# psmyth94/mamba-clip

Hardware: AMD Instinct MI355X
Metric: image-text pairs/sec (whole node) + selective_scan HBM GB/s (higher is better)
Workload: dtype bf16; 1 GPU; C2: ViT-B/16 image + Mamba-130M text, contrastive train step (fwd+bwd+AdamW), amp_bf16; model=vit_b16-mamba130m, global_batch=256, per_gpu_batch=256, seq_len=77, image_size=224, input=resident, step_launch=eager, parallelism=dp1, library_gemm_selection=tunableop-file

## Files before the change

### include/mc_ops.h

```cpp
#ifndef MAMBA_CLIP_AMD_MC_OPS_H
#define MAMBA_CLIP_AMD_MC_OPS_H

#include <stddef.h>
#include <stdint.h>

#include "mc_scan.h"

#ifdef __cplusplus
extern "C" {
#endif

int mc_add_rmsnorm_fwd(int32_t rows, int32_t cols, int32_t dtype, const void* x, const float* res_in, const float* w,
                       float eps, void* y, float* res_out, float* rstd, void* stream);

int mc_add_rmsnorm_bwd(int32_t rows, int32_t cols, int32_t dtype, const void* dy, const float* dres, const float* h,
                       const float* w, const float* rstd, void* dx, float* dres_in, float* dw, void* workspace,
                       size_t workspace_bytes, void* stream);
size_t mc_add_rmsnorm_bwd_workspace_bytes(int32_t rows, int32_t cols);

int mc_last_token_rmsnorm_fwd(int32_t batch, int32_t T, int32_t Lp, int32_t cols, int32_t dtype, const int64_t* tokens,
                              int64_t pad_id, const void* x, const float* res_in, const float* w, float eps, void* y,
                              float* h_out, float* rstd, int32_t* pos, void* stream);

int mc_last_token_rmsnorm_bwd(int32_t batch, int32_t Lp, int32_t cols, int32_t dtype, const void* dy, const float* h,
// ... 29 lines not shown
  const float* scale;
  const float* shift;
  void* out;
} mc_patch_input_params;
int mc_patch_embed_input(const mc_patch_input_params* p, void* stream);

size_t mc_grad_colsum_workspace_bytes(int32_t rows, int32_t cols);
int mc_gelu_bwd(int32_t rows, int32_t cols, int32_t dtype, const void* h, int64_t ldh, const void* ga, int64_t ldga,
                void* gh, int64_t ldgh, float* dbias, void* workspace, size_t workspace_bytes, void* stream);

typedef struct mc_qkv_pack_params {
  int32_t batch, seq, heads, head_dim, dtype;
  const void* src[3];
  int64_t sb[3], sn[3], sh[3];
  void* out; int64_t ld_out;
  float* dbias;
  void* workspace; size_t workspace_bytes;
} mc_qkv_pack_params;
int mc_qkv_grad_pack(const mc_qkv_pack_params* p, void* stream);

int mc_stream_copy(const void* src, void* dst, size_t nbytes, void* stream);

int mc_sum_slabs(int32_t s, int64_t n, const float* src, int64_t slab_stride, float* dst, void* stream);

#define MC_CAST_CHUNK 16384
typedef struct {
  const float* src;
  int64_t dst_off;
  int64_t n;
} mc_cast_chunk;
int mc_cast_f32_many(int32_t n_chunks, const mc_cast_chunk* chunks, void* dst_base, int32_t dst_dtype, void* stream);

typedef struct mc_cast_t_tile {
  const float* src;
  int64_t dst_off;
  int32_t src_ld, dst_ld;
  int32_t rows, cols;
} mc_cast_t_tile;
int mc_cast_transpose_f32_many(int32_t n_tiles, const mc_cast_t_tile* tiles, void* dst_base, int32_t dst_dtype,
                               void* stream);

#define MC_ADAMW_MAX_GROUPS 8
#define MC_ADAMW_CHUNK 65536
typedef struct mc_adamw_tensor {
  float* p;
  float* m;
  float* v;
  const float* g;
} mc_adamw_tensor;
typedef struct mc_adamw_chunk {
  int32_t tensor, group;
  int64_t off, n;
} mc_adamw_chunk;
typedef struct mc_adamw_group {
  float beta1, beta2, eps, decay;
  float step_size, bc2_sqrt;
} mc_adamw_group;
typedef struct mc_adamw_hyper {
  int32_t n_groups, reserved;
  mc_adamw_group group[MC_ADAMW_MAX_GROUPS];
} mc_adamw_hyper;
int mc_adamw_step(int32_t n_chunks, const mc_adamw_chunk* chunks, const mc_adamw_tensor* tensors,
                  const mc_adamw_hyper* hyper, void* stream);

size_t mc_colsum_workspace_bytes(int32_t rows, int32_t cols);
int mc_colsum(int32_t rows, int32_t cols, int32_t dtype, const void* x, int64_t ld, float* out,
              void* workspace, size_t workspace_bytes, void* stream);
int mc_colsum_fold(int32_t nslices, int32_t cols, const float* part, float* out, void* stream);

int mc_l2norm_fwd(int32_t rows, int32_t cols, int32_t dtype, const void* x, int64_t ldx, float eps,
                  float* y, int64_t ldy, float* norm, void* stream);
int mc_l2norm_bwd(int32_t rows, int32_t cols, int32_t dtype, const void* x, int64_t ldx, const float* norm,
                  float eps, const float* g, int64_t ldg, void* dx, int64_t lddx, void* stream);

#ifdef __cplusplus
}
#endif
#endif
```

### mamba-clip_amd/csrc/ops.hip

```cpp
#include <algorithm>

#include "mc_common.h"
#include "../../include/mc_ops.h"

namespace mc {

namespace ops {

constexpr int kMaxVec = 8;

template <int V>
__device__ __forceinline__ void ld_f32v(const float* __restrict__ p, float (&v)[V]) {
#pragma unroll
  for (int e4 = 0; e4 < V; e4 += 4) {
    const float4 q = *reinterpret_cast<const float4*>(p + e4);
    v[e4] = q.x; v[e4 + 1] = q.y; v[e4 + 2] = q.z; v[e4 + 3] = q.w;
  }
}
template <int V>
__device__ __forceinline__ void st_f32v(float* __restrict__ p, const float (&v)[V]) {
#pragma unroll
  for (int e4 = 0; e4 < V; e4 += 4)
    *reinterpret_cast<float4*>(p + e4) = make_float4(v[e4], v[e4 + 1], v[e4 + 2], v[e4 + 3]);
}

template <int V>
__device__ __forceinline__ void fold_stage(float (&red)[3][64 * V], const float (&acc)[V], int lane) {
  const int w = threadIdx.x >> 6;
  if (w > 0) {
#pragma unroll
    for (int e = 0; e < V; ++e) red[w - 1][lane * V + e] = acc[e];
  }
  __syncthreads();
// ... 1356 lines not shown
  if (vec) {
    for (int64_t i = 8 * (int64_t)threadIdx.x; i < c.n; i += 8 * 256) {
      const float4 a = *reinterpret_cast<const float4*>(c.src + i);
      const float4 b = *reinterpret_cast<const float4*>(c.src + i + 4);
      const float v[8] = {a.x, a.y, a.z, a.w, b.x, b.y, b.z, b.w};
      *reinterpret_cast<uint4*>(dst + i) = pack_f<TO>(v);
    }
  } else {
    for (int64_t i = threadIdx.x; i < c.n; i += 256) dst[i] = from_f<TO>(c.src[i]);
  }
}
}

extern "C" int mc_cast_f32_many(int32_t n_chunks, const mc_cast_chunk* chunks, void* dst_base, int32_t dst_dtype,
                                void* stream) {
  MC_CHECK(n_chunks >= 0 && (n_chunks == 0 || (chunks && dst_base)), MC_ERR_INVALID, "mc_cast_f32_many: bad chunk table");
  MC_CHECK(dst_dtype == MC_DTYPE_BF16 || dst_dtype == MC_DTYPE_F16, MC_ERR_DTYPE,
           "mc_cast_f32_many: dst dtype %d (bf16 / f16 only)", dst_dtype);
  if (n_chunks == 0) return MC_OK;
  if (dst_dtype == MC_DTYPE_BF16)
    hipLaunchKernelGGL(cast_many_kernel<bf16_t>, dim3(n_chunks), dim3(256), 0, (hipStream_t)stream, chunks,
                       reinterpret_cast<bf16_t*>(dst_base));
  else
    hipLaunchKernelGGL(cast_many_kernel<f16_t>, dim3(n_chunks), dim3(256), 0, (hipStream_t)stream, chunks,
                       reinterpret_cast<f16_t*>(dst_base));
  return check_launch("mc_cast_f32_many");
}

namespace {
template <typename TO>
__global__ __launch_bounds__(256) void cast_transpose_kernel(const mc_cast_t_tile* __restrict__ tiles, TO* __restrict__ base) {
  __shared__ float tile[64][65];
  const mc_cast_t_tile t = tiles[blockIdx.x];
  const int tid = threadIdx.x, r = tid >> 2, a = tid & 3;
  const bool full = t.rows == 64 && t.cols == 64 && (t.src_ld & 3) == 0 && (reinterpret_cast<uintptr_t>(t.src) & 15) == 0;
  if (full) {
    float4 v[4];
#pragma unroll
    for (int k = 0; k < 4; ++k) v[k] = *reinterpret_cast<const float4*>(t.src + (int64_t)r * t.src_ld + 4 * (a + 4 * k));
#pragma unroll
    for (int k = 0; k < 4; ++k) {
      const int c = 4 * (a + 4 * k);
      tile[r][c] = v[k].x; tile[r][c + 1] = v[k].y; tile[r][c + 2] = v[k].z; tile[r][c + 3] = v[k].w;
    }
  } else {
#pragma unroll
    for (int k = 0; k < 4; ++k)
#pragma unroll
      for (int e = 0; e < 4; ++e) {
        const int c = 4 * (a + 4 * k) + e;
        tile[r][c] = (r < t.rows && c < t.cols) ? t.src[(int64_t)r * t.src_ld + c] : 0.f;
      }
  }
  __syncthreads();
  const int j = tid >> 2;
  TO* dst = base + t.dst_off + (int64_t)j * t.dst_ld;
  const bool vec = full && (t.dst_ld & 7) == 0 && (reinterpret_cast<uintptr_t>(base + t.dst_off) & 15) == 0;
#pragma unroll
  for (int hlf = 0; hlf < 2; ++hlf) {
    const int g = a + 4 * hlf;
    float v[8];
#pragma unroll
    for (int e = 0; e < 8; ++e) v[e] = tile[8 * g + e][j];
    if (vec) {
      *reinterpret_cast<uint4*>(dst + 8 * g) = pack_f<TO>(v);
    } else if (j < t.cols) {
#pragma unroll
      for (int e = 0; e < 8; ++e)
        if (8 * g + e < t.rows) dst[8 * g + e] = from_f<TO>(v[e]);
    }
  }
}
}

extern "C" int mc_cast_transpose_f32_many(int32_t n_tiles, const mc_cast_t_tile* tiles, void* dst_base, int32_t dst_dtype,
                                          void* stream) {
  MC_CHECK(n_tiles >= 0 && (n_tiles == 0 || (tiles && dst_base)), MC_ERR_INVALID, "mc_cast_transpose_f32_many: bad tile table");
  MC_CHECK(dst_dtype == MC_DTYPE_BF16 || dst_dtype == MC_DTYPE_F16, MC_ERR_DTYPE,
           "mc_cast_transpose_f32_many: dst dtype %d (bf16 / f16 only)", dst_dtype);
  if (n_tiles == 0) return MC_OK;
  if (dst_dtype == MC_DTYPE_BF16)
    hipLaunchKernelGGL(cast_transpose_kernel<bf16_t>, dim3(n_tiles), dim3(256), 0, (hipStream_t)stream, tiles,
                       reinterpret_cast<bf16_t*>(dst_base));
  else
    hipLaunchKernelGGL(cast_transpose_kernel<f16_t>, dim3(n_tiles), dim3(256), 0, (hipStream_t)stream, tiles,
                       reinterpret_cast<f16_t*>(dst_base));
  return check_launch("mc_cast_transpose_f32_many");
}

namespace {
__device__ __forceinline__ void adamw_elem(float& p, float& m, float& v, float g, const mc_adamw_group& h) {
  p *= h.decay;
  m = h.beta1 * m + (1.f - h.beta1) * g;
  v = h.beta2 * v + (1.f - h.beta2) * g * g;
  const float denom = sqrtf(v) / h.bc2_sqrt + h.eps;
  p -= h.step_size * m / denom;
}

__global__ __launch_bounds__(256) void adamw_kernel(const mc_adamw_chunk* __restrict__ chunks,
                                                    const mc_adamw_tensor* __restrict__ tensors, const mc_adamw_hyper hy) {
  const mc_adamw_chunk c = chunks[blockIdx.x];
  const mc_adamw_tensor t = tensors[c.tensor];
  const mc_adamw_group h = hy.group[c.group];
  float* __restrict__ p = t.p + c.off;
  float* __restrict__ m = t.m + c.off;
  float* __restrict__ v = t.v + c.off;
  const float* __restrict__ g = t.g + c.off;
  const bool vec = ((reinterpret_cast<uintptr_t>(p) | reinterpret_cast<uintptr_t>(m) | reinterpret_cast<uintptr_t>(v) |
                     reinterpret_cast<uintptr_t>(g)) & 15) == 0;
  const int64_t n4 = vec ? c.n / 4 : 0;
  for (int64_t i = threadIdx.x; i < n4; i += 256) {
    float4 pp = reinterpret_cast<float4*>(p)[i], mm = reinterpret_cast<float4*>(m)[i];
    float4 vv = reinterpret_cast<float4*>(v)[i];
    const float4 gg = reinterpret_cast<const float4*>(g)[i];
    adamw_elem(pp.x, mm.x, vv.x, gg.x, h);
    adamw_elem(pp.y, mm.y, vv.y, gg.y, h);
    adamw_elem(pp.z, mm.z, vv.z, gg.z, h);
    adamw_elem(pp.w, mm.w, vv.w, gg.w, h);
    reinterpret_cast<float4*>(p)[i] = pp;
    reinterpret_cast<float4*>(m)[i] = mm;
    reinterpret_cast<float4*>(v)[i] = vv;
  }
  for (int64_t i = 4 * n4 + threadIdx.x; i < c.n; i += 256) {
    float pp = p[i], mm = m[i], vv = v[i];
    adamw_elem(pp, mm, vv, g[i], h);
    p[i] = pp;
    m[i] = mm;
    v[i] = vv;
  }
}
}

extern "C" int mc_adamw_step(int32_t n_chunks, const mc_adamw_chunk* chunks, const mc_adamw_tensor* tensors,
                             const mc_adamw_hyper* hyper, void* stream) {
  MC_CHECK(n_chunks >= 0 && hyper, MC_ERR_INVALID, "mc_adamw_step: bad arguments");
  MC_CHECK(hyper->n_groups >= 1 && hyper->n_groups <= MC_ADAMW_MAX_GROUPS, MC_ERR_INVALID,
           "mc_adamw_step: n_groups %d (1..%d)", hyper->n_groups, MC_ADAMW_MAX_GROUPS);
  if (n_chunks == 0) return MC_OK;
  MC_CHECK(chunks && tensors, MC_ERR_INVALID, "mc_adamw_step: null chunk / tensor table");
  hipLaunchKernelGGL(adamw_kernel, dim3(n_chunks), dim3(256), 0, (hipStream_t)stream, chunks, tensors, *hyper);
  return check_launch("mc_adamw_step");
}

namespace {
template <bool kVec>
__global__ __launch_bounds__(256) void sum_slabs_kernel(int s, int64_t n, const float* __restrict__ src, int64_t stride,
                                                        float* __restrict__ dst) {
  const int64_t i0 = ((int64_t)blockIdx.x * 256 + threadIdx.x) * (kVec ? 4 : 1);
  if (i0 >= n) return;
  if constexpr (kVec) {
    float4 acc = *reinterpret_cast<const float4*>(src + i0);
    for (int k = 1; k < s; ++k) {
      const float4 v = *reinterpret_cast<const float4*>(src + (int64_t)k * stride + i0);
      acc.x += v.x; acc.y += v.y; acc.z += v.z; acc.w += v.w;
    }
    *reinterpret_cast<float4*>(dst + i0) = acc;
  } else {
    float acc = src[i0];
    for (int k = 1; k < s; ++k) acc += src[(int64_t)k * stride + i0];
    dst[i0] = acc;
  }
}
}

extern "C" int mc_sum_slabs(int32_t s, int64_t n, const float* src, int64_t slab_stride, float* dst, void* stream) {
  MC_CHECK(s >= 1 && n >= 0 && slab_stride >= n, MC_ERR_SHAPE, "mc_sum_slabs: bad shape (s %d, n %lld, stride %lld)", s,
           (long long)n, (long long)slab_stride);
  if (n == 0) return MC_OK;
  MC_CHECK(src && dst, MC_ERR_INVALID, "mc_sum_slabs: null pointer");
  const bool vec = n % 4 == 0 && slab_stride % 4 == 0 && aligned16(src) && aligned16(dst);
  const int64_t items = vec ? n / 4 : n;
  const dim3 grid((unsigned)((items + 255) / 256));
  if (vec) hipLaunchKernelGGL(sum_slabs_kernel<true>, grid, dim3(256), 0, (hipStream_t)stream, s, n, src, slab_stride, dst);
  else hipLaunchKernelGGL(sum_slabs_kernel<false>, grid, dim3(256), 0, (hipStream_t)stream, s, n, src, slab_stride, dst);
// ... 69 lines not shown
```

### mamba-clip_amd/mamba_clip_amd/_lib.py

```python
import ctypes
import os

_HERE = os.path.dirname(os.path.abspath(__file__))
LIB_PATH = os.environ.get("MAMBA_CLIP_AMD_LIB") or os.path.join(_HERE, "libmamba_clip_amd.so")

MC_DTYPE_F32, MC_DTYPE_BF16, MC_DTYPE_F16, MC_DTYPE_FP8_E4M3, MC_DTYPE_U8 = 0, 1, 2, 3, 4
MC_LAYOUT_NCHW, MC_LAYOUT_NHWC = 0, 1
MC_SCAN_CHUNK = 32
MC_SCAN_STATE_INTERVAL_FINE = 8
MC_SCAN_KERNEL_NONE, MC_SCAN_KERNEL_PAIR, MC_SCAN_KERNEL_GENERIC, MC_SCAN_KERNEL_DIRS = 0, 1, 2, 3
MC_GEMM_KERNEL_TILE, MC_GEMM_KERNEL_FP8_TILE, MC_GEMM_KERNEL_FP8_PANEL = 1, 2, 3
MC_SCAN_MAX_DSTATE = 32
MC_CAST_CHUNK = 16384

c_i32, c_i64, c_vp, c_fp = ctypes.c_int32, ctypes.c_int64, ctypes.c_void_p, ctypes.c_void_p


class ScanFwdParams(ctypes.Structure):
    _fields_ = [
        ("batch", c_i32), ("dim", c_i32), ("seqlen", c_i32), ("dstate", c_i32), ("n_groups", c_i32),
        ("itype", c_i32), ("wtype", c_i32), ("delta_softplus", c_i32),
        ("u_batch_stride", c_i64), ("u_dim_stride", c_i64),
        ("delta_batch_stride", c_i64), ("delta_dim_stride", c_i64),
        ("z_batch_stride", c_i64), ("z_dim_stride", c_i64),
# ... 238 lines not shown
    "mc_retrieval_ranks_workspace_bytes": (ctypes.c_size_t, [c_i32, c_i32]),
    "mc_sigmoid_loss_fwd": (ctypes.c_int, [ctypes.POINTER(SigmoidLossParams), c_vp]),
    "mc_sigmoid_loss_fwd_workspace_bytes": (ctypes.c_size_t, [c_i32, c_i32]),
    "mc_sigmoid_loss_grad": (ctypes.c_int, [ctypes.POINTER(SigmoidLossParams), c_vp]),
    "mc_sigmoid_loss_grad_workspace_bytes": (ctypes.c_size_t, [c_i32, c_i32]),
    "mc_add_rmsnorm_fwd": (ctypes.c_int, [c_i32, c_i32, c_i32, c_vp, c_fp, c_fp, ctypes.c_float, c_vp, c_fp, c_fp,
                                          c_vp]),
    "mc_add_rmsnorm_bwd": (ctypes.c_int, [c_i32, c_i32, c_i32, c_vp, c_fp, c_fp, c_fp, c_fp, c_vp, c_fp, c_fp, c_vp,
                                          ctypes.c_size_t, c_vp]),
    "mc_add_rmsnorm_bwd_workspace_bytes": (ctypes.c_size_t, [c_i32, c_i32]),
    "mc_last_token_rmsnorm_fwd": (ctypes.c_int, [c_i32, c_i32, c_i32, c_i32, c_i32, c_vp, c_i64, c_vp, c_fp, c_fp,
                                                 ctypes.c_float, c_vp, c_fp, c_fp, c_vp, c_vp]),
    "mc_last_token_rmsnorm_bwd": (ctypes.c_int, [c_i32, c_i32, c_i32, c_i32, c_vp, c_fp, c_fp, c_fp, c_vp, c_vp, c_fp,
                                                 c_fp, c_vp]),
    "mc_add_layernorm_fwd": (ctypes.c_int, [c_i32, c_i32, c_i32, c_vp, c_vp, c_fp, c_fp, ctypes.c_float, c_vp, c_vp,
                                            c_fp, c_fp, c_vp]),
    "mc_add_layernorm_bwd": (ctypes.c_int, [c_i32, c_i32, c_i32, c_vp, c_vp, c_vp, c_fp, c_fp, c_fp, c_vp, c_fp, c_fp,
                                            c_fp, c_vp, ctypes.c_size_t, c_vp]),
    "mc_add_layernorm_bwd_workspace_bytes": (ctypes.c_size_t, [c_i32, c_i32]),
    "mc_causal_conv1d_fwd": (ctypes.c_int, [c_i32, c_i32, c_i32, c_i32, c_i32, c_vp, c_i64, c_i64, c_fp, c_fp, c_i32,
                                            c_vp, c_i64, c_i64, c_vp]),
    "mc_causal_conv1d_bwd": (ctypes.c_int, [c_i32, c_i32, c_i32, c_i32, c_i32, c_vp, c_i64, c_i64, c_fp, c_fp, c_i32,
                                            c_vp, c_i64, c_i64, c_vp, c_i64, c_i64, c_fp, c_fp, c_vp,
                                            ctypes.c_size_t, c_vp]),
    "mc_causal_conv1d_bwd_workspace_bytes": (ctypes.c_size_t, [c_i32, c_i32, c_i32, c_i32]),
    "mc_patch_im2col": (ctypes.c_int, [c_i32, c_i32, c_i32, c_i32, c_i32, c_i32, c_vp, c_vp, c_vp]),
    "mc_grad_colsum_workspace_bytes": (ctypes.c_size_t, [c_i32, c_i32]),
    "mc_gelu_bwd": (ctypes.c_int, [c_i32, c_i32, c_i32, c_vp, c_i64, c_vp, c_i64, c_vp, c_i64, c_fp, c_vp,
                                   ctypes.c_size_t, c_vp]),
    "mc_qkv_grad_pack": (ctypes.c_int, [ctypes.POINTER(QkvPackParams), c_vp]),
    "mc_stream_copy": (ctypes.c_int, [c_vp, c_vp, ctypes.c_size_t, c_vp]),
    "mc_cast_f32_many": (ctypes.c_int, [c_i32, c_vp, c_vp, c_i32, c_vp]),
    "mc_cast_transpose_f32_many": (ctypes.c_int, [c_i32, c_vp, c_vp, c_i32, c_vp]),
    "mc_adamw_step": (ctypes.c_int, [c_i32, c_vp, c_vp, ctypes.POINTER(AdamWHyper), c_vp]),
    "mc_sum_slabs": (ctypes.c_int, [c_i32, c_i64, c_fp, c_i64, c_fp, c_vp]),
    "mc_colsum_workspace_bytes": (ctypes.c_size_t, [c_i32, c_i32]),
    "mc_colsum_fold": (ctypes.c_int, [c_i32, c_i32, c_fp, c_fp, c_vp]),
    "mc_colsum": (ctypes.c_int, [c_i32, c_i32, c_i32, c_vp, c_i64, c_fp, c_vp, ctypes.c_size_t, c_vp]),
    "mc_l2norm_fwd": (ctypes.c_int, [c_i32, c_i32, c_i32, c_vp, c_i64, ctypes.c_float, c_fp, c_i64, c_fp, c_vp]),
    "mc_l2norm_bwd": (ctypes.c_int, [c_i32, c_i32, c_i32, c_vp, c_i64, c_fp, ctypes.c_float, c_fp, c_i64, c_vp,
                                     c_i64, c_vp]),
    "mc_attn_fwd": (ctypes.c_int, [ctypes.POINTER(AttnFwdParams), c_vp]),
    "mc_attn_bwd": (ctypes.c_int, [ctypes.POINTER(AttnBwdParams), c_vp]),
    "mc_attn_masked_fwd": (ctypes.c_int, [ctypes.POINTER(AttnMaskedFwdParams), c_vp]),
    "mc_attn_masked_bwd": (ctypes.c_int, [ctypes.POINTER(AttnMaskedBwdParams), c_vp]),
    "mc_patch_embed_input": (ctypes.c_int, [ctypes.POINTER(PatchInputParams), c_vp]),
    "mc_ss2d_conv_stack_fwd": (ctypes.c_int, [ctypes.POINTER(SS2DConvParams), c_vp]),
    "mc_ss2d_conv_stack_bwd": (ctypes.c_int, [ctypes.POINTER(SS2DConvBwdParams), c_vp]),
    "mc_ss2d_conv_bwd_workspace_bytes": (ctypes.c_size_t, [c_i32, c_i32, c_i32, c_i32, c_i32]),
    "mc_ss2d_merge_ln_gate_fwd": (ctypes.c_int, [ctypes.POINTER(SS2DMergeParams), c_vp]),
    "mc_ss2d_merge_ln_gate_bwd": (ctypes.c_int, [ctypes.POINTER(SS2DMergeBwdParams), c_vp]),
    "mc_ss2d_merge_bwd_workspace_bytes": (ctypes.c_size_t, [c_i32, c_i32, c_i32, c_i32]),
    "mc_ss2d_group_proj": (ctypes.c_int, [ctypes.POINTER(SS2DGroupProjParams), c_vp]),
}

_lib = None


def load():
    global _lib
    if _lib is not None:
        return _lib
    if not os.path.exists(LIB_PATH):
        raise ImportError(
            f"mamba_clip_amd: HIP library not found at {LIB_PATH}; build it with "
            "`make -C mamba-clip_amd` (gfx950).  There is no CPU fallback.")
    import torch
# ... 32 lines not shown
```

### mamba-clip_amd/mamba_clip_amd/ops.py

```python
import collections
import ctypes
import weakref

import torch

from . import _lib


def _ws(nbytes, device):
    return torch.empty(max(int(nbytes), 16), dtype=torch.uint8, device=device)


def gemm_nt(A, B, alpha=1.0, alpha_dev=None, out_dtype=torch.float32, scale_a=None, scale_b=None, out=None):
    lib = _lib.load()
    if A.dtype != B.dtype or A.dtype not in (torch.bfloat16, torch.float32, torch.float8_e4m3fn):
        raise RuntimeError("gemm_nt: A and B must both be bf16, both fp32 or both float8_e4m3fn")
    if A.stride(-1) != 1:
        A = A.contiguous()
    if B.stride(-1) != 1:
        B = B.contiguous()
    M, K = A.shape
    N, K2 = B.shape
    if K != K2:
        raise RuntimeError("gemm_nt: inner dimensions differ")
# ... 918 lines not shown
        ctx.save_for_backward(*outs)
        ctx.set_materialize_grads(False)
        return tuple(outs)

    @staticmethod
    def backward(ctx, *gs):
        outs = ctx.saved_tensors
        idx = [i for i, g in enumerate(gs) if g is not None]
        res = [None] * len(gs)
        if idx:
            for i, v in zip(idx, torch._foreach_mul([gs[i].float() for i in idx], [outs[i] for i in idx])):
                res[i] = v
        return tuple(res)


def neg_exp_many(logs):
    return list(NegExpManyFn.apply(*logs))


class GradHandoff:

    def __init__(self):
        self.du = None

    def take(self):
        du, self.du = self.du, None
        return du


_WCAST = None
_WCAST_T = None
_T_WANTED = weakref.WeakValueDictionary()
_CAST_PLANS = {}


def _wcast(t, dt):
    if t.dtype == dt:
        return t
    if _WCAST is not None:
        e = _WCAST.get(id(t))
        if e is not None and e[0] is t and e[1].dtype == dt:
            return e[1]
    return t.to(dt)


class _CastPlan:

    def __init__(self, params, dt, device):
        offs, off = [], 0
        rows = []
        for p in params:
            offs.append(off)
            n = p.numel()
            for s0 in range(0, n, _lib.MC_CAST_CHUNK):
                rows.append((p.data_ptr() + 4 * s0, off + s0, min(_lib.MC_CAST_CHUNK, n - s0)))
            off += (n + 7) // 8 * 8
        self.offs, self.total, self.dt = offs, off, dt
        self.nchunks = len(rows)
        self.table = torch.tensor(rows, dtype=torch.int64).to(device)

    def run(self, params):
        buf = torch.empty(self.total, device=self.table.device, dtype=self.dt)
        _lib.check(_lib.load().mc_cast_f32_many(self.nchunks, self.table.data_ptr(), buf.data_ptr(),
                                                _lib.dtype_code(self.dt), _lib.stream_handle(buf.device)),
                   "mc_cast_f32_many")
        return [buf[o:o + p.numel()].view(p.shape) for o, p in zip(self.offs, params)]


def _wcast_t(weight, x, dt):
    if not (x.is_cuda and weight.dim() == 2 and weight.numel() >= 1 << 19
            and x.numel() // max(x.shape[-1], 1) >= 8192):
        return None
    if _WCAST_T is not None:
        e = _WCAST_T.get(id(weight))
        if e is not None and e[0] is weight and e[1].dtype == dt:
            return e[1]
    if _WCAST is not None and weight.dtype == torch.float32:
        _T_WANTED[id(weight)] = weight
    return None


class _TransposePlan:

    def __init__(self, params, dt, device):
        offs, off, rows = [], 0, []
        for p in params:
            R, C = p.shape
            offs.append(off)
            for r0 in range(0, R, 64):
                for c0 in range(0, C, 64):
                    rows.append((p.data_ptr() + 4 * (r0 * C + c0), off + c0 * R + r0,
                                 C | (R << 32), min(64, R - r0) | (min(64, C - c0) << 32)))
            off += (R * C + 7) // 8 * 8
        self.offs, self.total, self.dt = offs, off, dt
        self.ntiles = len(rows)
        self.table = torch.tensor(rows, dtype=torch.int64).to(device)

    def run(self, params):
        buf = torch.empty(self.total, device=self.table.device, dtype=self.dt)
        _lib.check(_lib.load().mc_cast_transpose_f32_many(self.ntiles, self.table.data_ptr(), buf.data_ptr(),
                                                          _lib.dtype_code(self.dt), _lib.stream_handle(buf.device)),
                   "mc_cast_transpose_f32_many")
        return [buf[o:o + p.numel()].view(p.shape[1], p.shape[0]) for o, p in zip(self.offs, params)]


class weight_cast_scope:

    def __init__(self, module, dt):
        self.module, self.dt, self.active = module, dt, False

    def __enter__(self):
        global _WCAST, _WCAST_T
        if _WCAST is not None or self.dt not in (torch.bfloat16, torch.float16):
            return self
        params = [p for m in self.module.modules() if isinstance(m, torch.nn.Linear)
                  for p in (m.weight, m.bias)
                  if p is not None and p.is_cuda and p.dtype == torch.float32 and p.is_contiguous()]
        if not params:
            return self
        key = (id(self.module), self.dt, tuple((p.data_ptr(), p.numel()) for p in params))
        plan = _CAST_PLANS.get(key[:2])
        if plan is None or plan[0] != key:
            plan = (key, _CastPlan(params, self.dt, params[0].device))
            _CAST_PLANS[key[:2]] = plan
        copies = plan[1].run(params)
        _WCAST = {id(p): (p, c) for p, c in zip(params, copies)}
        tparams = [p for p in params if p.dim() == 2 and _T_WANTED.get(id(p)) is p]
        if tparams:
            tkey = (id(self.module), self.dt, "t", tuple((p.data_ptr(), p.shape) for p in tparams))
            tplan = _CAST_PLANS.get(tkey[:3])
            if tplan is None or tplan[0] != tkey:
                tplan = (tkey, _TransposePlan(tparams, self.dt, params[0].device))
                _CAST_PLANS[tkey[:3]] = tplan
            tcopies = tplan[1].run(tparams)
            _WCAST_T = {id(p): (p, c) for p, c in zip(tparams, tcopies)}
        self.active = True
        return self

    def __exit__(self, *exc):
        global _WCAST, _WCAST_T
        if self.active:
            _WCAST = _WCAST_T = None
        return False


def _dgrad(g2, wc, wt=None):
    if wt is not None:
        return torch.mm(g2, wt.t())
    if g2.is_cuda and g2.shape[0] >= 8192 and wc.shape[0] * wc.shape[1] >= 1 << 19:
        return torch.mm(g2, wc.t().contiguous().t())
    return torch.mm(g2, wc)


def _compute_dtype(t):
    if t.is_cuda and torch.is_autocast_enabled("cuda"):
        return torch.get_autocast_dtype("cuda")
    return t.dtype


class LinearSK(torch.autograd.Function):

    @staticmethod
    def forward(ctx, x, weight, bias):
        dt = _compute_dtype(x)
        xc, wc = x.to(dt), _wcast(weight, dt)
# ... 616 lines not shown
```

### mamba-clip_amd/mamba_clip_amd/optim.py

```python
import math

import torch

from . import _lib


class HipAdamW(torch.optim.Optimizer):
    def __init__(self, params, lr=1e-3, betas=(0.9, 0.999), eps=1e-8, weight_decay=1e-2):
        if not 0.0 <= lr or not 0.0 <= eps or not 0.0 <= betas[0] < 1.0 or not 0.0 <= betas[1] < 1.0:
            raise ValueError(f"HipAdamW: invalid hyper-parameters lr={lr} betas={betas} eps={eps}")
        super().__init__(params, dict(lr=lr, betas=betas, eps=eps, weight_decay=weight_decay, amsgrad=False,
                                      maximize=False, foreach=None, capturable=False, differentiable=False,
                                      fused=None, decoupled_weight_decay=True))
        self._plans = {}

    def _share_steps(self):
        for group in self.param_groups:
            shared = {}
            for p in group["params"]:
                s = self.state.get(p)
                if s is None or "step" not in s:
                    continue
                t = float(s["step"])
                if t not in shared:
                    shared[t] = torch.tensor(t, dtype=torch.float32)
                s["step"] = shared[t]

    def load_state_dict(self, state_dict):
        super().load_state_dict(state_dict)
        self._share_steps()
        self._plans = {}

    def state_dict(self):
        sd = super().state_dict()
        sd["state"] = {k: dict(v, step=v["step"].clone()) if "step" in v else v for k, v in sd["state"].items()}
        return sd

    def _advance_steps(self, group, ps):
        movers = {}
        fresh = []
        for p in ps:
            s = self.state[p]
            if "exp_avg" not in s:
                s["exp_avg"] = torch.zeros_like(p, memory_format=torch.preserve_format)
                s["exp_avg_sq"] = torch.zeros_like(p, memory_format=torch.preserve_format)
            st = s.get("step")
            if st is None:
                fresh.append(s)
            else:
                movers.setdefault(id(st), (st, []))[1].append(s)
        if fresh:
            one = torch.tensor(1.0, dtype=torch.float32)
            for s in fresh:
                s["step"] = one
        if not movers:
            return
        holders = {}
        for p in group["params"]:
            st = self.state.get(p, {}).get("step")
            if st is not None and id(st) in movers:
                holders[id(st)] = holders.get(id(st), 0) + 1
        for key, (st, states) in movers.items():
            if len(states) == holders[key]:
                st += 1.0
            else:
                nxt = st + 1.0
                for s in states:
                    s["step"] = nxt

    @staticmethod
    def _build_plan(live, dev):
        chunks, tensors = [], []
        for ti, (bi, p, s) in enumerate(live):
            n = p.numel()
            for off in range(0, n, _lib.MC_ADAMW_CHUNK):
                chunks.append((ti | (bi << 32), off, min(_lib.MC_ADAMW_CHUNK, n - off)))
            tensors.append((p.data_ptr(), s["exp_avg"].data_ptr(), s["exp_avg_sq"].data_ptr()))
        return dict(n=len(chunks), chunks=torch.tensor(chunks, dtype=torch.int64).to(dev), base=tensors)

    @torch.no_grad()
    def step(self, closure=None):
        loss = None
        if closure is not None:
            with torch.enable_grad():
                loss = closure()
        buckets = {}
        for gi, group in enumerate(self.param_groups):
            if group.get("amsgrad") or group.get("maximize") or not group.get("decoupled_weight_decay", True):
                raise RuntimeError("HipAdamW: amsgrad / maximize / coupled weight decay are not supported")
            ps = [p for p in group["params"] if p.grad is not None]
            for p in ps:
                if p.grad.is_sparse:
                    raise RuntimeError("HipAdamW does not support sparse gradients")
                if not (p.is_cuda and p.dtype == torch.float32 and p.is_contiguous()
                        and p.grad.dtype == torch.float32 and p.grad.is_contiguous()):
                    raise RuntimeError("HipAdamW: fp32 contiguous CUDA parameters and gradients only")
            self._advance_steps(group, ps)
            for p in ps:
                s = self.state[p]
                buckets.setdefault((gi, float(s["step"])), []).append((p, s))
        if not buckets:
            return loss
        keys = list(buckets)
        per = _lib.MC_ADAMW_MAX_GROUPS
        for b0 in range(0, len(keys), per):
            self._launch([(k, buckets[k]) for k in keys[b0:b0 + per]])
        return loss

    def _launch(self, bucket_list):
        hyper = _lib.AdamWHyper()
        hyper.n_groups = len(bucket_list)
        live = []
        for bi, ((gi, t), members) in enumerate(bucket_list):
            group = self.param_groups[gi]
            b1, b2 = group["betas"]
            h = hyper.group[bi]
            h.beta1, h.beta2, h.eps = b1, b2, group["eps"]
            h.decay = 1.0 - group["lr"] * group["weight_decay"]
            h.step_size = group["lr"] / (1.0 - b1 ** t)
            h.bc2_sqrt = math.sqrt(1.0 - b2 ** t)
            live.extend((bi, p, s) for p, s in members)
        dev = live[0][1].device
        key = tuple((bi, id(p), p.data_ptr(), id(s["exp_avg"])) for bi, p, s in live)
        plan = self._plans.get(key)
        if plan is None:
            if len(self._plans) > 16:
                self._plans.clear()
            plan = self._plans[key] = self._build_plan(live, dev)
        rows = [b + (p.grad.data_ptr(),) for b, (_, p, _) in zip(plan["base"], live)]
        tens = torch.tensor(rows, dtype=torch.int64).pin_memory().to(dev, non_blocking=True)
        _lib.check(_lib.load().mc_adamw_step(plan["n"], plan["chunks"].data_ptr(), tens.data_ptr(), hyper,
                                             _lib.stream_handle(dev)), "mc_adamw_step")
        plan["tens"] = tens
```

Measured before the change: 3766 image-text pairs/sec.

## Emit bf16 weight shadows from AdamW and reuse them for forward casts

The AdamW kernel now also writes a low-precision copy of each updated parameter into a persistent shadow buffer. The forward-pass weight cast then reuses these shadows instead of re-reading fp32 weights and casting them again. Transposed weight copies are built by a new 16-bit transpose kernel that reads the shadows instead of cast-transposing from fp32. This removes a separate fp32 read and cast pass per step, at the cost of extra shadow memory and version-tracking bookkeeping that must stay correct when parameters change outside the optimizer.

```diff
diff --git a/include/mc_ops.h b/include/mc_ops.h
--- a/include/mc_ops.h
+++ b/include/mc_ops.h
@@ -85,13 +85,14 @@
 int mc_cast_f32_many(int32_t n_chunks, const mc_cast_chunk* chunks, void* dst_base, int32_t dst_dtype, void* stream);
 
 typedef struct mc_cast_t_tile {
-  const float* src;
+  const void* src;
   int64_t dst_off;
   int32_t src_ld, dst_ld;
   int32_t rows, cols;
 } mc_cast_t_tile;
 int mc_cast_transpose_f32_many(int32_t n_tiles, const mc_cast_t_tile* tiles, void* dst_base, int32_t dst_dtype,
                                void* stream);
+int mc_transpose16_many(int32_t n_tiles, const mc_cast_t_tile* tiles, void* dst_base, int32_t dtype, void* stream);
 
 #define MC_ADAMW_MAX_GROUPS 8
 #define MC_ADAMW_CHUNK 65536
@@ -115,6 +116,8 @@
 } mc_adamw_hyper;
 int mc_adamw_step(int32_t n_chunks, const mc_adamw_chunk* chunks, const mc_adamw_tensor* tensors,
                   const mc_adamw_hyper* hyper, void* stream);
+int mc_adamw_step_shadow(int32_t n_chunks, const mc_adamw_chunk* chunks, const mc_adamw_tensor* tensors,
+                         void* const* shadows, int32_t shadow_dtype, const mc_adamw_hyper* hyper, void* stream);
 
 size_t mc_colsum_workspace_bytes(int32_t rows, int32_t cols);
 int mc_colsum(int32_t rows, int32_t cols, int32_t dtype, const void* x, int64_t ld, float* out,
diff --git a/mamba-clip_amd/csrc/ops.hip b/mamba-clip_amd/csrc/ops.hip
--- a/mamba-clip_amd/csrc/ops.hip
+++ b/mamba-clip_amd/csrc/ops.hip
@@ -1,4 +1,5 @@
 #include <algorithm>
+#include <type_traits>
 
 #include "mc_common.h"
 #include "../../include/mc_ops.h"
@@ -1421,12 +1422,13 @@
 __global__ __launch_bounds__(256) void cast_transpose_kernel(const mc_cast_t_tile* __restrict__ tiles, TO* __restrict__ base) {
   __shared__ float tile[64][65];
   const mc_cast_t_tile t = tiles[blockIdx.x];
+  const float* __restrict__ src = static_cast<const float*>(t.src);
   const int tid = threadIdx.x, r = tid >> 2, a = tid & 3;
-  const bool full = t.rows == 64 && t.cols == 64 && (t.src_ld & 3) == 0 && (reinterpret_cast<uintptr_t>(t.src) & 15) == 0;
+  const bool full = t.rows == 64 && t.cols == 64 && (t.src_ld & 3) == 0 && (reinterpret_cast<uintptr_t>(src) & 15) == 0;
   if (full) {
     float4 v[4];
 #pragma unroll
-    for (int k = 0; k < 4; ++k) v[k] = *reinterpret_cast<const float4*>(t.src + (int64_t)r * t.src_ld + 4 * (a + 4 * k));
+    for (int k = 0; k < 4; ++k) v[k] = *reinterpret_cast<const float4*>(src + (int64_t)r * t.src_ld + 4 * (a + 4 * k));
 #pragma unroll
     for (int k = 0; k < 4; ++k) {
       const int c = 4 * (a + 4 * k);
@@ -1438,7 +1440,7 @@
 #pragma unroll
       for (int e = 0; e < 4; ++e) {
         const int c = 4 * (a + 4 * k) + e;
-        tile[r][c] = (r < t.rows && c < t.cols) ? t.src[(int64_t)r * t.src_ld + c] : 0.f;
+        tile[r][c] = (r < t.rows && c < t.cols) ? src[(int64_t)r * t.src_ld + c] : 0.f;
       }
   }
   __syncthreads();
@@ -1460,6 +1462,67 @@
     }
   }
 }
+
+__global__ __launch_bounds__(256) void transpose16_kernel(const mc_cast_t_tile* __restrict__ tiles,
+                                                          uint16_t* __restrict__ base) {
+  __shared__ uint16_t tile[64][66];
+  const mc_cast_t_tile t = tiles[blockIdx.x];
+  const uint16_t* __restrict__ src = static_cast<const uint16_t*>(t.src);
+  const int tid = threadIdx.x, r = tid >> 2, a = tid & 3;
+  const bool full = t.rows == 64 && t.cols == 64 && (t.src_ld & 7) == 0 && (reinterpret_cast<uintptr_t>(src) & 15) == 0;
+  if (full) {
+    uint4 v[2];
+#pragma unroll
+    for (int k = 0; k < 2; ++k) v[k] = *reinterpret_cast<const uint4*>(src + (int64_t)r * t.src_ld + 8 * (a + 4 * k));
+#pragma unroll
+    for (int k = 0; k < 2; ++k) {
+      const int c = 8 * (a + 4 * k);
+#pragma unroll
+      for (int w = 0; w < 4; ++w) {
+        const uint32_t x = word_of(v[k], w);
+        tile[r][c + 2 * w] = (uint16_t)(x & 0xffffu);
+        tile[r][c + 2 * w + 1] = (uint16_t)(x >> 16);
+      }
+    }
+  } else {
+#pragma unroll
+    for (int k = 0; k < 2; ++k)
+#pragma unroll
+      for (int e = 0; e < 8; ++e) {
+        const int c = 8 * (a + 4 * k) + e;
+        tile[r][c] = (r < t.rows && c < t.cols) ? src[(int64_t)r * t.src_ld + c] : (uint16_t)0;
+      }
+  }
+  __syncthreads();
+  const int j = tid >> 2;
+  uint16_t* dst = base + t.dst_off + (int64_t)j * t.dst_ld;
+  const bool vec = full && (t.dst_ld & 7) == 0 && (reinterpret_cast<uintptr_t>(base + t.dst_off) & 15) == 0;
+#pragma unroll
+  for (int hlf = 0; hlf < 2; ++hlf) {
+    const int g = a + 4 * hlf;
+    uint32_t v[8];
+#pragma unroll
+    for (int e = 0; e < 8; ++e) v[e] = tile[8 * g + e][j];
+    if (vec) {
+      *reinterpret_cast<uint4*>(dst + 8 * g) =
+          make_uint4(v[0] | (v[1] << 16), v[2] | (v[3] << 16), v[4] | (v[5] << 16), v[6] | (v[7] << 16));
+    } else if (j < t.cols) {
+#pragma unroll
+      for (int e = 0; e < 8; ++e)
+        if (8 * g + e < t.rows) dst[8 * g + e] = (uint16_t)v[e];
+    }
+  }
+}
+}
+
+extern "C" int mc_transpose16_many(int32_t n_tiles, const mc_cast_t_tile* tiles, void* dst_base, int32_t dtype, void* stream) {
+  MC_CHECK(n_tiles >= 0 && (n_tiles == 0 || (tiles && dst_base)), MC_ERR_INVALID, "mc_transpose16_many: bad tile table");
+  MC_CHECK(dtype == MC_DTYPE_BF16 || dtype == MC_DTYPE_F16, MC_ERR_DTYPE, "mc_transpose16_many: dtype %d (bf16 / f16 only)",
+           dtype);
+  if (n_tiles == 0) return MC_OK;
+  hipLaunchKernelGGL(transpose16_kernel,dim3(n_tiles), dim3(256), 0, (hipStream_t)stream, tiles,
+                     reinterpret_cast<uint16_t*>(dst_base));
+  return check_launch("mc_transpose16_many");
 }
 
 extern "C" int mc_cast_transpose_f32_many(int32_t n_tiles, const mc_cast_t_tile* tiles, void* dst_base, int32_t dst_dtype,
@@ -1486,11 +1549,9 @@
   p -= h.step_size * m / denom;
 }
 
-__global__ __launch_bounds__(256) void adamw_kernel(const mc_adamw_chunk* __restrict__ chunks,
-                                                    const mc_adamw_tensor* __restrict__ tensors, const mc_adamw_hyper hy) {
-  const mc_adamw_chunk c = chunks[blockIdx.x];
-  const mc_adamw_tensor t = tensors[c.tensor];
-  const mc_adamw_group h = hy.group[c.group];
+template <typename TS>
+__device__ __forceinline__ void adamw_chunk(const mc_adamw_chunk& c, const mc_adamw_tensor& t, void* shadow,
+                                            const mc_adamw_group& h) {
   float* __restrict__ p = t.p + c.off;
   float* __restrict__ m = t.m + c.off;
   float* __restrict__ v = t.v + c.off;
@@ -1498,37 +1559,115 @@
   const bool vec = ((reinterpret_cast<uintptr_t>(p) | reinterpret_cast<uintptr_t>(m) | reinterpret_cast<uintptr_t>(v) |
                      reinterpret_cast<uintptr_t>(g)) & 15) == 0;
   const int64_t n4 = vec ? c.n / 4 : 0;
-  for (int64_t i = threadIdx.x; i < n4; i += 256) {
-    float4 pp = reinterpret_cast<float4*>(p)[i], mm = reinterpret_cast<float4*>(m)[i];
-    float4 vv = reinterpret_cast<float4*>(v)[i];
-    const float4 gg = reinterpret_cast<const float4*>(g)[i];
-    adamw_elem(pp.x, mm.x, vv.x, gg.x, h);
-    adamw_elem(pp.y, mm.y, vv.y, gg.y, h);
-    adamw_elem(pp.z, mm.z, vv.z, gg.z, h);
-    adamw_elem(pp.w, mm.w, vv.w, gg.w, h);
-    reinterpret_cast<float4*>(p)[i] = pp;
-    reinterpret_cast<float4*>(m)[i] = mm;
-    reinterpret_cast<float4*>(v)[i] = vv;
-  }
-  for (int64_t i = 4 * n4 + threadIdx.x; i < c.n; i += 256) {
-    float pp = p[i], mm = m[i], vv = v[i];
-    adamw_elem(pp, mm, vv, g[i], h);
-    p[i] = pp;
-    m[i] = mm;
-    v[i] = vv;
-  }
+  if constexpr (std::is_void<TS>::value) {
+    for (int64_t i = threadIdx.x; i < n4; i += 256) {
+      float4 pp = reinterpret_cast<float4*>(p)[i], mm = reinterpret_cast<float4*>(m)[i];
+      float4 vv = reinterpret_cast<float4*>(v)[i];
+      const float4 gg = reinterpret_cast<const float4*>(g)[i];
+      adamw_elem(pp.x, mm.x, vv.x, gg.x, h);
+      adamw_elem(pp.y, mm.y, vv.y, gg.y, h);
+      adamw_elem(pp.z, mm.z, vv.z, gg.z, h);
+      adamw_elem(pp.w, mm.w, vv.w, gg.w, h);
+      reinterpret_cast<float4*>(p)[i] = pp;
+      reinterpret_cast<float4*>(m)[i] = mm;
+      reinterpret_cast<float4*>(v)[i] = vv;
+    }
+    for (int64_t i = 4 * n4 + threadIdx.x; i < c.n; i += 256) {
+      float pp = p[i], mm = m[i], vv = v[i];
+      adamw_elem(pp, mm, vv, g[i], h);
+      p[i] = pp;
+      m[i] = mm;
+      v[i] = vv;
+    }
+  } else {
+    TS* __restrict__ sh = shadow ? static_cast<TS*>(shadow) + c.off : nullptr;
+    const bool sh8 = (reinterpret_cast<uintptr_t>(sh) & 7) == 0;
+    for (int64_t i = threadIdx.x; i < n4; i += 256) {
+      float4 pp = reinterpret_cast<float4*>(p)[i], mm = reinterpret_cast<float4*>(m)[i];
+      float4 vv = reinterpret_cast<float4*>(v)[i];
+      const float4 gg = reinterpret_cast<const float4*>(g)[i];
+      adamw_elem(pp.x, mm.x, vv.x, gg.x, h);
+      adamw_elem(pp.y, mm.y, vv.y, gg.y, h);
+      adamw_elem(pp.z, mm.z, vv.z, gg.z, h);
+      adamw_elem(pp.w, mm.w, vv.w, gg.w, h);
+      reinterpret_cast<float4*>(p)[i] = pp;
+      reinterpret_cast<float4*>(m)[i] = mm;
+      reinterpret_cast<float4*>(v)[i] = vv;
+      if (sh) {
+        if (sh8) {
+          reinterpret_cast<uint2*>(sh)[i] = make_uint2(cvt_pk2<TS>(pp.x, pp.y), cvt_pk2<TS>(pp.z, pp.w));
+        } else {
+          sh[4 * i] = from_f<TS>(pp.x);
+          sh[4 * i + 1] = from_f<TS>(pp.y);
+          sh[4 * i + 2] = from_f<TS>(pp.z);
+          sh[4 * i + 3] = from_f<TS>(pp.w);
+        }
+      }
+    }
+    for (int64_t i = 4 * n4 + threadIdx.x; i < c.n; i += 256) {
+      float pp = p[i], mm = m[i], vv = v[i];
+      adamw_elem(pp, mm, vv, g[i], h);
+      p[i] = pp;
+      m[i] = mm;
+      v[i] = vv;
+    }
+    if (sh)
+      for (int64_t i = 4 * n4 + threadIdx.x; i < c.n; i += 256) sh[i] = from_f<TS>(p[i]);
+  }
+}
+
+__global__ __launch_bounds__(256) void adamw_kernel(const mc_adamw_chunk* __restrict__ chunks,
+                                                    const mc_adamw_tensor* __restrict__ tensors, const mc_adamw_hyper hy) {
+  const mc_adamw_chunk c = chunks[blockIdx.x];
+  const mc_adamw_tensor t = tensors[c.tensor];
+  const mc_adamw_group h = hy.group[c.group];
+  adamw_chunk<void>(c, t, nullptr, h);
+}
+
+template <typename TS>
+__global__ __launch_bounds__(256) void adamw_shadow_kernel(const mc_adamw_chunk* __restrict__ chunks,
+                                                           const mc_adamw_tensor* __restrict__ tensors,
+                                                           void* const* __restrict__ shadows, const mc_adamw_hyper hy) {
+  const mc_adamw_chunk c = chunks[blockIdx.x];
+  const mc_adamw_tensor t = tensors[c.tensor];
+  const mc_adamw_group h = hy.group[c.group];
+  adamw_chunk<TS>(c, t, shadows[c.tensor], h);
+}
+}
+
+namespace {
+int adamw_check(int32_t n_chunks, const mc_adamw_hyper* hyper, const char* who) {
+  MC_CHECK(n_chunks >= 0 && hyper, MC_ERR_INVALID, "%s: bad arguments", who);
+  MC_CHECK(hyper->n_groups >= 1 && hyper->n_groups <= MC_ADAMW_MAX_GROUPS, MC_ERR_INVALID, "%s: n_groups %d (1..%d)", who,
+           hyper->n_groups, MC_ADAMW_MAX_GROUPS);
+  return MC_OK;
 }
 }
 
 extern "C" int mc_adamw_step(int32_t n_chunks, const mc_adamw_chunk* chunks, const mc_adamw_tensor* tensors,
                              const mc_adamw_hyper* hyper, void* stream) {
-  MC_CHECK(n_chunks >= 0 && hyper, MC_ERR_INVALID, "mc_adamw_step: bad arguments");
-  MC_CHECK(hyper->n_groups >= 1 && hyper->n_groups <= MC_ADAMW_MAX_GROUPS, MC_ERR_INVALID,
-           "mc_adamw_step: n_groups %d (1..%d)", hyper->n_groups, MC_ADAMW_MAX_GROUPS);
+  if (const int rc = adamw_check(n_chunks, hyper, "mc_adamw_step")) return rc;
   if (n_chunks == 0) return MC_OK;
   MC_CHECK(chunks && tensors, MC_ERR_INVALID, "mc_adamw_step: null chunk / tensor table");
   hipLaunchKernelGGL(adamw_kernel, dim3(n_chunks), dim3(256), 0, (hipStream_t)stream, chunks, tensors, *hyper);
   return check_launch("mc_adamw_step");
+}
+
+extern "C" int mc_adamw_step_shadow(int32_t n_chunks, const mc_adamw_chunk* chunks, const mc_adamw_tensor* tensors,
+                                    void* const* shadows, int32_t shadow_dtype, const mc_adamw_hyper* hyper, void* stream) {
+  if (!shadows) return mc_adamw_step(n_chunks, chunks, tensors, hyper, stream);
+  if (const int rc = adamw_check(n_chunks, hyper, "mc_adamw_step_shadow")) return rc;
+  MC_CHECK(shadow_dtype == MC_DTYPE_BF16 || shadow_dtype == MC_DTYPE_F16, MC_ERR_DTYPE,
+           "mc_adamw_step_shadow: shadow dtype %d (bf16 / f16 only)", shadow_dtype);
+  if (n_chunks == 0) return MC_OK;
+  MC_CHECK(chunks && tensors, MC_ERR_INVALID, "mc_adamw_step_shadow: null chunk / tensor table");
+  if (shadow_dtype == MC_DTYPE_BF16)
+    hipLaunchKernelGGL(adamw_shadow_kernel<bf16_t>, dim3(n_chunks), dim3(256), 0, (hipStream_t)stream, chunks, tensors,
+                       shadows, *hyper);
+  else
+    hipLaunchKernelGGL(adamw_shadow_kernel<f16_t>, dim3(n_chunks), dim3(256), 0, (hipStream_t)stream, chunks, tensors,
+                       shadows, *hyper);
+  return check_launch("mc_adamw_step_shadow");
 }
 
 namespace {
diff --git a/mamba-clip_amd/mamba_clip_amd/_lib.py b/mamba-clip_amd/mamba_clip_amd/_lib.py
--- a/mamba-clip_amd/mamba_clip_amd/_lib.py
+++ b/mamba-clip_amd/mamba_clip_amd/_lib.py
@@ -294,7 +294,9 @@
     "mc_stream_copy": (ctypes.c_int, [c_vp, c_vp, ctypes.c_size_t, c_vp]),
     "mc_cast_f32_many": (ctypes.c_int, [c_i32, c_vp, c_vp, c_i32, c_vp]),
     "mc_cast_transpose_f32_many": (ctypes.c_int, [c_i32, c_vp, c_vp, c_i32, c_vp]),
+    "mc_transpose16_many": (ctypes.c_int, [c_i32, c_vp, c_vp, c_i32, c_vp]),
     "mc_adamw_step": (ctypes.c_int, [c_i32, c_vp, c_vp, ctypes.POINTER(AdamWHyper), c_vp]),
+    "mc_adamw_step_shadow": (ctypes.c_int, [c_i32, c_vp, c_vp, c_vp, c_i32, ctypes.POINTER(AdamWHyper), c_vp]),
     "mc_sum_slabs": (ctypes.c_int, [c_i32, c_i64, c_fp, c_i64, c_fp, c_vp]),
     "mc_colsum_workspace_bytes": (ctypes.c_size_t, [c_i32, c_i32]),
     "mc_colsum_fold": (ctypes.c_int, [c_i32, c_i32, c_fp, c_fp, c_vp]),
diff --git a/mamba-clip_amd/mamba_clip_amd/ops.py b/mamba-clip_amd/mamba_clip_amd/ops.py
--- a/mamba-clip_amd/mamba_clip_amd/ops.py
+++ b/mamba-clip_amd/mamba_clip_amd/ops.py
@@ -974,6 +974,28 @@
 _WCAST_T = None
 _T_WANTED = weakref.WeakValueDictionary()
 _CAST_PLANS = {}
+_SHADOW_WANTED = weakref.WeakValueDictionary()
+_SHADOW_DT = None
+_SHADOW_GEN = 0
+_SHADOW = {}
+
+
+def want_shadows(params, dt):
+    global _SHADOW_DT, _SHADOW_GEN
+    if _SHADOW_DT != dt:
+        _SHADOW_DT = dt
+        _SHADOW_GEN += 1
+    for p in params:
+        if _SHADOW_WANTED.get(id(p)) is not p:
+            _SHADOW_WANTED[id(p)] = p
+            _SHADOW_GEN += 1
+
+
+def shadow_of(p, dt):
+    e = _SHADOW.get(id(p))
+    if e is not None and e[0]() is p and e[1].dtype == dt and e[2] == p.data_ptr() and e[3] == p._version:
+        return e[1]
+    return None
 
 
 def _wcast(t, dt):
@@ -1024,25 +1046,27 @@
 
 class _TransposePlan:
 
-    def __init__(self, params, dt, device):
+    def __init__(self, params, dt, device, sources=None):
         offs, off, rows = [], 0, []
-        for p in params:
+        for i, p in enumerate(params):
             R, C = p.shape
             offs.append(off)
+            base, esz = (p.data_ptr(), 4) if sources is None else (sources[i].data_ptr(), 2)
             for r0 in range(0, R, 64):
                 for c0 in range(0, C, 64):
-                    rows.append((p.data_ptr() + 4 * (r0 * C + c0), off + c0 * R + r0,
+                    rows.append((base + esz * (r0 * C + c0), off + c0 * R + r0,
                                  C | (R << 32), min(64, R - r0) | (min(64, C - c0) << 32)))
             off += (R * C + 7) // 8 * 8
         self.offs, self.total, self.dt = offs, off, dt
         self.ntiles = len(rows)
         self.table = torch.tensor(rows, dtype=torch.int64).to(device)
+        self.from16 = sources is not None
 
     def run(self, params):
         buf = torch.empty(self.total, device=self.table.device, dtype=self.dt)
-        _lib.check(_lib.load().mc_cast_transpose_f32_many(self.ntiles, self.table.data_ptr(), buf.data_ptr(),
-                                                          _lib.dtype_code(self.dt), _lib.stream_handle(buf.device)),
-                   "mc_cast_transpose_f32_many")
+        fn = "mc_transpose16_many" if self.from16 else "mc_cast_transpose_f32_many"
+        _lib.check(getattr(_lib.load(), fn)(self.ntiles, self.table.data_ptr(), buf.data_ptr(),
+                                            _lib.dtype_code(self.dt), _lib.stream_handle(buf.device)), fn)
         return [buf[o:o + p.numel()].view(p.shape[1], p.shape[0]) for o, p in zip(self.offs, params)]
 
 
@@ -1060,19 +1084,33 @@
                   if p is not None and p.is_cuda and p.dtype == torch.float32 and p.is_contiguous()]
         if not params:
             return self
-        key = (id(self.module), self.dt, tuple((p.data_ptr(), p.numel()) for p in params))
-        plan = _CAST_PLANS.get(key[:2])
-        if plan is None or plan[0] != key:
-            plan = (key, _CastPlan(params, self.dt, params[0].device))
-            _CAST_PLANS[key[:2]] = plan
-        copies = plan[1].run(params)
-        _WCAST = {id(p): (p, c) for p, c in zip(params, copies)}
+        served = {}
+        if _SHADOW and not torch.cuda.is_current_stream_capturing():
+            for p in params:
+                c = shadow_of(p, self.dt)
+                if c is not None:
+                    served[id(p)] = c
+        miss = [p for p in params if id(p) not in served] if served else params
+        copies = {id(p): (p, served[id(p)]) for p in params if id(p) in served}
+        if miss:
+            want_shadows(miss, self.dt)
+            key = (id(self.module), self.dt, tuple((p.data_ptr(), p.numel()) for p in miss))
+            plan = _CAST_PLANS.get(key[:2])
+            if plan is None or plan[0] != key:
+                plan = (key, _CastPlan(miss, self.dt, miss[0].device))
+                _CAST_PLANS[key[:2]] = plan
+            copies.update({id(p): (p, c) for p, c in zip(miss, plan[1].run(miss))})
+        _WCAST = copies
         tparams = [p for p in params if p.dim() == 2 and _T_WANTED.get(id(p)) is p]
         if tparams:
-            tkey = (id(self.module), self.dt, "t", tuple((p.data_ptr(), p.shape) for p in tparams))
+            src = [served.get(id(p)) for p in tparams]
+            if any(c is None for c in src):
+                src = None
+            tkey = (id(self.module), self.dt, "t",
+                    tuple((t.data_ptr(), p.shape) for t, p in zip(src or tparams, tparams)), src is None)
             tplan = _CAST_PLANS.get(tkey[:3])
             if tplan is None or tplan[0] != tkey:
-                tplan = (tkey, _TransposePlan(tparams, self.dt, params[0].device))
+                tplan = (tkey, _TransposePlan(tparams, self.dt, params[0].device, src))
                 _CAST_PLANS[tkey[:3]] = tplan
             tcopies = tplan[1].run(tparams)
             _WCAST_T = {id(p): (p, c) for p, c in zip(tparams, tcopies)}
diff --git a/mamba-clip_amd/mamba_clip_amd/optim.py b/mamba-clip_amd/mamba_clip_amd/optim.py
--- a/mamba-clip_amd/mamba_clip_amd/optim.py
+++ b/mamba-clip_amd/mamba_clip_amd/optim.py
@@ -1,18 +1,20 @@
 import math
+import weakref
 
 import torch
 
-from . import _lib
+from . import _lib, ops
 
 
 class HipAdamW(torch.optim.Optimizer):
-    def __init__(self, params, lr=1e-3, betas=(0.9, 0.999), eps=1e-8, weight_decay=1e-2):
+    def __init__(self, params, lr=1e-3, betas=(0.9, 0.999), eps=1e-8, weight_decay=1e-2, shadows=True):
         if not 0.0 <= lr or not 0.0 <= eps or not 0.0 <= betas[0] < 1.0 or not 0.0 <= betas[1] < 1.0:
             raise ValueError(f"HipAdamW: invalid hyper-parameters lr={lr} betas={betas} eps={eps}")
         super().__init__(params, dict(lr=lr, betas=betas, eps=eps, weight_decay=weight_decay, amsgrad=False,
                                       maximize=False, foreach=None, capturable=False, differentiable=False,
                                       fused=None, decoupled_weight_decay=True))
         self._plans = {}
+        self._shadows = shadows
 
     def _share_steps(self):
         for group in self.param_groups:
@@ -68,15 +70,30 @@
                 for s in states:
                     s["step"] = nxt
 
-    @staticmethod
-    def _build_plan(live, dev):
+    def _build_plan(self, live, dev):
         chunks, tensors = [], []
         for ti, (bi, p, s) in enumerate(live):
             n = p.numel()
             for off in range(0, n, _lib.MC_ADAMW_CHUNK):
                 chunks.append((ti | (bi << 32), off, min(_lib.MC_ADAMW_CHUNK, n - off)))
             tensors.append((p.data_ptr(), s["exp_avg"].data_ptr(), s["exp_avg_sq"].data_ptr()))
-        return dict(n=len(chunks), chunks=torch.tensor(chunks, dtype=torch.int64).to(dev), base=tensors)
+        plan = dict(n=len(chunks), chunks=torch.tensor(chunks, dtype=torch.int64).to(dev), base=tensors, shadow=None)
+        dt = ops._SHADOW_DT
+        wanted = [p for _, p, _ in live if ops._SHADOW_WANTED.get(id(p)) is p] if self._shadows and dt is not None else []
+        if wanted:
+            offs, off = {}, 0
+            for p in wanted:
+                offs[id(p)] = off
+                off += (p.numel() + 7) // 8 * 8
+            buf = torch.empty(off, device=dev, dtype=dt)
+            ptrs = [buf.data_ptr() + 2 * offs[id(p)] if id(p) in offs else 0 for _, p, _ in live]
+            entries = []
+            for p in wanted:
+                e = [None, buf[offs[id(p)]:offs[id(p)] + p.numel()].view(p.shape), 0, -1]
+                e[0] = weakref.ref(p, lambda _, k=id(p), e=e: ops._SHADOW.get(k) is e and ops._SHADOW.pop(k))
+                entries.append(e)
+            plan["shadow"] = dict(buf=buf, ptrs=torch.tensor(ptrs, dtype=torch.int64).to(dev), dt=dt, entries=entries)
+        return plan
 
     @torch.no_grad()
     def step(self, closure=None):
@@ -121,7 +138,8 @@
             h.bc2_sqrt = math.sqrt(1.0 - b2 ** t)
             live.extend((bi, p, s) for p, s in members)
         dev = live[0][1].device
-        key = tuple((bi, id(p), p.data_ptr(), id(s["exp_avg"])) for bi, p, s in live)
+        key = (ops._SHADOW_GEN if self._shadows else -1,) + \
+            tuple((bi, id(p), p.data_ptr(), id(s["exp_avg"])) for bi, p, s in live)
         plan = self._plans.get(key)
         if plan is None:
             if len(self._plans) > 16:
@@ -129,6 +147,17 @@
             plan = self._plans[key] = self._build_plan(live, dev)
         rows = [b + (p.grad.data_ptr(),) for b, (_, p, _) in zip(plan["base"], live)]
         tens = torch.tensor(rows, dtype=torch.int64).pin_memory().to(dev, non_blocking=True)
-        _lib.check(_lib.load().mc_adamw_step(plan["n"], plan["chunks"].data_ptr(), tens.data_ptr(), hyper,
-                                             _lib.stream_handle(dev)), "mc_adamw_step")
+        sh = plan["shadow"]
+        if sh is None:
+            _lib.check(_lib.load().mc_adamw_step(plan["n"], plan["chunks"].data_ptr(), tens.data_ptr(), hyper,
+                                                 _lib.stream_handle(dev)), "mc_adamw_step")
+        else:
+            _lib.check(_lib.load().mc_adamw_step_shadow(plan["n"], plan["chunks"].data_ptr(), tens.data_ptr(),
+                                                        sh["ptrs"].data_ptr(), _lib.dtype_code(sh["dt"]), hyper,
+                                                        _lib.stream_handle(dev)), "mc_adamw_step_shadow")
+            torch.autograd.graph.increment_version(sh["buf"])
+            for e in sh["entries"]:
+                p = e[0]()
+                e[2], e[3] = p.data_ptr(), p._version
+                ops._SHADOW[id(p)] = e
         plan["tens"] = tens
```

After: 3774 image-text pairs/sec (median of 6 runs). About the same (+0.2%).
